# maxvonbuelow/harry

Hardware: AMD Instinct MI355X
Metric: Mtriangles/s encode+decode (higher is better)
Workload: dtype u8/u16 residual bytes, u32 range-coder registers (compat profile: u64)

## Files before the change

### harry_amd/csrc/device/chunked.cpp

```cpp
#include <chrono>
#include <condition_variable>
#include <cstdio>
#include <cstdlib>
#include <cstring>
#include <deque>
#include <memory>
#include <mutex>
#include <thread>

#include "codec_math.hpp"
#include "context.hpp"
#include "kernels.hpp"

namespace hry {

using namespace dev;
static const char kMarkPrefix[] = "[hry enc]";

static constexpr int kDefaultChunk = 8192;
static constexpr uint32_t kMaxChunk = 1u << 20;


static uint32_t stream_words(uint32_t n, uint32_t t0)
{
// ... 526 lines not shown
	shard_arrays_ready();
	const bool piped = pipe && pipe->began;
	if (pipe) { pipe->finish(); w.progress = nullptr; }
	if (piped) HRY_MARK(t_all, "  pipeline drained");
	ChunkedDirectory dir;
	std::vector<uint8_t> restart_sec;
	auto select_restarts = [&] {
		std::vector<RestartCounters> scounters;
		dir.restarts = select_restart_points(w.marks, w.named, dir.counters, &w.snapshots, &scounters);
		if (!w.snapshots.empty()) write_snapshot_section(w.snapshot_faces, w.snapshots, scounters, dir.snapshot_section);
		write_restart_section(dir, restart_sec);
	};
	const bool dir_beside = w.marks.size() >= 4096 && host_threads() > 1;
	SideThreads dir_helper;
	if (dir_beside) dir_helper.spawn(select_restarts);

	const uint32_t vc = (uint32_t)w.order_v.size(), fc = (uint32_t)w.order_f.size();
	if (piped && (vc != pipe->vc || fc != pipe->fc)) throw Error(HRY_E_INTERNAL, "encode pipeline: sizes changed under the walk");
	if (chunk_syms <= 0) {
		uint64_t total = (uint64_t)w.n_conn + (uint64_t)vc * ldv.nplanes + (uint64_t)fc * ldf.nplanes;
		if (m.general) for (const AttrList &L : m.lists) total += (uint64_t)L.count * L.coded_bytes();
		while (CH < (1u << 15) && total / CH > 8192) CH <<= 1;
	}

	auto t_h2d = Clock::now();
	size_t op_plane_n[8];
	for (int k = 0; k < 8; ++k) op_plane_n[k] = w.n_op_class[k];
	size_t ngrp = 0, conn_plane_bytes = 0, nopb = w.op_sc.size();
	for (int g = 0; g < G_COUNT; ++g) { ngrp += w.grp_val[g].size(); conn_plane_bytes += w.grp_val[g].size() * kGroupBytes[g]; }
	cx.d_order_v.ensure(std::max<size_t>((size_t)vc * 4, 16));
	cx.d_order_f.ensure(std::max<size_t>((size_t)fc * 4, 16));
	cx.d_rank.ensure(std::max<size_t>((size_t)dev_nv * 4, 16));
	cx.d_grp_val.ensure(std::max<size_t>(ngrp * 4, 16));
	cx.d_connplanes.ensure(std::max<size_t>(conn_plane_bytes + 2 * nopb + 64, 16));
	cx.d_vplanes.ensure(std::max<size_t>((size_t)vc * ldv.nplanes, 16));
	cx.d_fplanes.ensure(std::max<size_t>((size_t)fc * ldf.nplanes, 16));
	const bool nt_piped = piped && pipe->nt != nullptr;
	if (vc && !piped) HIP_OK(hipMemcpyAsync(cx.d_order_v.p, w.order_v.data(), (size_t)vc * 4, hipMemcpyHostToDevice, cx.stream));
	if (fc && (ldf.nplanes || m.general) && !piped) HIP_OK(hipMemcpyAsync(cx.d_order_f.p, w.order_f.data(), (size_t)fc * 4, hipMemcpyHostToDevice, cx.stream));
	if (!piped) upload_repaired_twins(cx, in_place ? *in_place->whole : m, w, in_place != nullptr);
	if (in_place) cx.inplace_twin_patches.insert(cx.inplace_twin_patches.end(), w.twin_patches.begin(), w.twin_patches.end());
	size_t goff[G_COUNT + 1] = { 0 };
	for (int g = 0; g < G_COUNT; ++g) {
		size_t n = w.grp_val[g].size();
		goff[g + 1] = goff[g] + n;
		if (n && !(g == G_NUMTRI && nt_piped)) HIP_OK(hipMemcpyAsync(cx.d_grp_val.as<uint32_t>() + goff[g], w.grp_val[g].data(), n * 4, hipMemcpyHostToDevice, cx.stream));
	}
	uint8_t *d_opplanes = cx.d_connplanes.as<uint8_t>() + conn_plane_bytes;
	uint8_t *d_opraw = d_opplanes + nopb;
	if (nopb) HIP_OK(hipMemcpyAsync(d_opraw, w.op_sc.data(), nopb, hipMemcpyHostToDevice, cx.stream));

	const std::vector<GenPlane> layout = container_planes(m);
	std::vector<PlaneRef> planes;
	auto add_plane = [&](const uint8_t *at, uint32_t n) { planes.push_back(PlaneRef{ at, n, layout.at(planes.size()).init }); };
	{
		size_t poff = 0;
		for (int g = 0; g < G_COUNT; ++g) {
			uint32_t n = (uint32_t)w.grp_val[g].size();
			const uint8_t *at = g == G_NUMTRI && nt_piped ? cx.d_nt_planes.as<uint8_t>() : cx.d_connplanes.as<uint8_t>() + poff;
			for (int b = 0; b < kGroupBytes[g]; ++b) add_plane(at + (size_t)b * n, n);
			poff += (size_t)n * kGroupBytes[g];
		}
		size_t o = 0;
		for (int k = 0; k < kOpClasses; ++k) { add_plane(d_opplanes + o, (uint32_t)op_plane_n[k]); o += op_plane_n[k]; }
		for (int p = 0; p < ldv.nplanes; ++p) add_plane(cx.d_vplanes.as<uint8_t>() + (size_t)p * vc, vc);
		for (int p = 0; p < ldf.nplanes; ++p) add_plane(cx.d_fplanes.as<uint8_t>() + (size_t)p * fc, fc);
	}
	if (m.general) general_planes_encode(cx, m, w, planes);
	if (planes.size() != layout.size()) throw Error(HRY_E_INTERNAL, "chunked encode: the planes do not match the container's layout");
	std::vector<uint32_t> kind_tabs;
	build_init_tables(m, kind_tabs);
	const uint32_t CHC = std::min(CH, std::max(CH / 8, 512u));
	dir.CH = CH; dir.CHC = CHC;
	const uint32_t npl = (uint32_t)planes.size();
	std::vector<HistSlice> slices;
	for (uint32_t pi = 0; pi < npl; ++pi)
		for (uint32_t f = 0; f < planes[pi].n; f += 16384) slices.push_back(HistSlice{ planes[pi].dptr + f, std::min(16384u, planes[pi].n - f), pi });
	cx.d_small.ensure(std::max<size_t>(slices.size() * sizeof(HistSlice) + (size_t)npl * 1024 + 64, 64));
	uint32_t *d_hist = cx.d_small.as<uint32_t>();
	HistSlice *d_slices = (HistSlice*)(cx.d_small.as<uint8_t>() + (size_t)npl * 1024);
	if (!slices.empty()) HIP_OK(hipMemcpyAsync(d_slices, slices.data(), slices.size() * sizeof(HistSlice), hipMemcpyHostToDevice, cx.stream));
	HIP_OK(hipMemsetAsync(d_hist, 0, (size_t)npl * 1024, cx.stream));
	HIP_OK(hipStreamSynchronize(cx.stream));
	cx.timing.h2d_ms = ms_since(t_h2d);
	HRY_MARK(t_all, "walk's outputs on the device");

	ConnView cv = cx.conn_view();
	HIP_OK(hipEventRecord(cx.ev[1], cx.stream));
	if (!m.general && !piped) {
		HIP_OK(hipMemsetAsync(cx.d_rank.p, 0xff, (size_t)dev_nv * 4, cx.stream));
		launch_rank(cx.stream, cx.d_order_v.as<uint32_t>(), vc, cv.org, cx.d_rank.as<uint32_t>());
		launch_predict_vtx(cx.stream, cv, cx.d_order_v.as<uint32_t>(), vc, cx.d_rank.as<uint32_t>(), cx.d_rec[1].as<uint8_t>(), ldv, cx.d_vplanes.as<uint8_t>());
		launch_face_planes(cx.stream, cv, cx.d_order_f.as<uint32_t>(), fc, cx.d_rec[0].as<uint8_t>(), ldf, cx.d_fplanes.as<uint8_t>());
	}
	split_conn_groups(cx, w, !nt_piped);
	{
		uint32_t base[8], o = 0;
		for (int k = 0; k < 8; ++k) { base[k] = o; o += (uint32_t)op_plane_n[k]; }
		cx.d_op.ensure(((nopb + kSplitUnit - 1) / kSplitUnit + 1) * 8 * 4 + 64);
		launch_split_classes(cx.stream, d_opraw, (uint32_t)nopb, base, cx.d_op.as<uint32_t>(), d_opplanes);
	}
	launch_plane_hist(cx.stream, d_slices, (uint32_t)slices.size(), d_hist);
	HIP_OK(hipEventRecord(cx.ev[2], cx.stream));
	std::vector<uint32_t> hist((size_t)npl * 256);
	if (npl) HIP_OK(hipMemcpyAsync(hist.data(), d_hist, hist.size() * 4, hipMemcpyDeviceToHost, cx.stream));
	HIP_OK(hipStreamSynchronize(cx.stream));
	HRY_MARK(t_all, "planes and their histograms");

	dir.tables.assign((size_t)npl * 256, 0);
	dir.has_prior.assign(npl, 0);
	dir.nsym.resize(npl);
	std::vector<uint32_t> totals(npl, 0);
	for (uint32_t pi = 0; pi < npl; ++pi) {
		uint32_t *tab = dir.tables.data() + (size_t)pi * 256;
		const bool use = plane_prior_from_hist(hist.data() + (size_t)pi * 256, planes[pi].n, tab);
		if (!use) memcpy(tab, kind_tabs.data() + (size_t)planes[pi].init * 256, 1024);
		for (int i = 0; i < 256; ++i) totals[pi] += tab[i];
		dir.has_prior[pi] = use ? 1 : 0;
		dir.nsym[pi] = planes[pi].n;
	}
	std::vector<StreamJob> jobs;
	uint64_t words = 0;
	uint64_t nsym_total = 0;
	uint32_t max_t0 = 256;
	for (uint32_t pi = 0; pi < npl; ++pi) {
		const PlaneRef &pl = planes[pi];
		nsym_total += pl.n;
		max_t0 = std::max(max_t0, totals[pi]);
		for_plane_streams(pi, pl.n, CH, CHC, [&](uint64_t f, uint32_t n) {
			if (words >= (1ull << 32) - (1u << 24)) throw Error(HRY_E_UNSUPPORTED, "chunked stream accumulator exceeds 2^32 words");
			jobs.push_back(StreamJob{ pl.dptr + f, n, pi, totals[pi], (uint32_t)words });
			words += stream_words(n, totals[pi]);
		});
	}
	const uint32_t ns = (uint32_t)jobs.size();
	const uint32_t nw = (uint32_t)words + 2;
	HRY_MARK(t_all, "  priors and stream jobs (host)");
	cx.d_init.ensure(std::max<size_t>(dir.tables.size() * 4, 16));
	if (!dir.tables.empty()) HIP_OK(hipMemcpyAsync(cx.d_init.p, dir.tables.data(), dir.tables.size() * 4, hipMemcpyHostToDevice, cx.stream));
	cx.d_cjobs.ensure(std::max<size_t>((size_t)ns * sizeof(StreamJob), 16));
	if (ns) HIP_OK(hipMemcpyAsync(cx.d_cjobs.p, jobs.data(), (size_t)ns * sizeof(StreamJob), hipMemcpyHostToDevice, cx.stream));
	cx.ensure_magic(max_t0 + CH + 16);
	cx.d_acc.ensure((size_t)nw * 8);
	cx.d_summary.ensure(((size_t)nw / 1024 + 8) * 4);
	cx.d_bytes.ensure((size_t)nw * 4);
	cx.d_csizes.ensure(std::max<size_t>((size_t)ns * 8, 16));
	cx.d_coffs.ensure(((size_t)ns + 1) * 8);
	HIP_OK(hipMemsetAsync(cx.d_acc.p, 0, (size_t)nw * 8, cx.stream));
	uint32_t *d_bits = cx.d_csizes.as<uint32_t>(), *d_nbytes = d_bits + ns;
	bool split_kernels;
	{
		uint32_t longest = 0;
		for (uint32_t i = 0; i < ns; ++i) longest = std::max(longest, jobs[i].n);
		const double one = std::max(longest * 0.09e-3, (double)nsym_total * 0.04e-6), two = longest * 0.207e-3 + (double)nsym_total * 0.0057e-6;
		const uint64_t min_streams = env_uint("HRY_ENCODE_SPLIT_MIN_STREAMS", ~0ull);
		split_kernels = min_streams != ~0ull ? min_streams != 0 && ns >= min_streams : ns >= 64 && two < 0.9 * one;
	}
	for (uint32_t i = 0; i < ns && split_kernels; ++i) split_kernels = (uint64_t)jobs[i].t0 + jobs[i].n <= 65535u;
	std::vector<uint64_t> tab;
	if (split_kernels) {
		tab.resize((size_t)ns + ((size_t)ns + 1) / 2);
		uint32_t *order = (uint32_t*)(tab.data() + ns);
		uint64_t off = 0;
		for (uint32_t i = 0; i < ns; ++i) { tab[i] = off; off += jobs[i].n; order[i] = i; }
		std::stable_sort(order, order + ns, [&](uint32_t a, uint32_t b) { return jobs[a].n > jobs[b].n; });
		cx.d_rec_sym.ensure(std::max<size_t>((size_t)off * 8, 16));
		cx.d_split.ensure(tab.size() * 8);
		HIP_OK(hipMemcpyAsync(cx.d_split.p, tab.data(), tab.size() * 8, hipMemcpyHostToDevice, cx.stream));
		HIP_OK(hipEventRecord(cx.ev[3], cx.stream));
		launch_chunk_encode_split(cx.stream, cx.d_cjobs.as<StreamJob>(), ns, cx.d_init.as<uint32_t>(), cx.d_magic.as<MagicEnt>(), cx.d_acc.as<uint64_t>(), d_bits,
		                          cx.d_split.as<uint64_t>(), cx.d_rec_sym.p, (const uint32_t*)(cx.d_split.as<uint64_t>() + ns));
		HIP_OK(hipEventRecord(cx.ev[4], cx.stream));
	} else {
	HIP_OK(hipEventRecord(cx.ev[3], cx.stream));
	launch_chunk_encode(cx.stream, cx.d_cjobs.as<StreamJob>(), ns, cx.d_init.as<uint32_t>(), cx.d_magic.as<MagicEnt>(), cx.d_acc.as<uint64_t>(), d_bits);
	HIP_OK(hipEventRecord(cx.ev[4], cx.stream));
	}
	launch_carry(cx.stream, cx.d_acc.as<uint64_t>(), nw, cx.d_v.as<uint64_t>(), cx.d_summary.as<uint32_t>(), cx.d_bytes.as<uint8_t>(), cx.d_cjobs.as<StreamJob>(), d_bits, ns);
	launch_stream_pack(cx.stream, cx.d_cjobs.as<StreamJob>(), ns, d_bits, nullptr, d_nbytes, cx.d_coffs.as<uint64_t>(), nullptr, false);
	cx.h_small.ensure(64);
	volatile uint64_t *total_bytes_p = cx.h_small.as<uint64_t>();
	*total_bytes_p = 0;
	HIP_OK(hipMemcpyAsync((void*)total_bytes_p, cx.d_coffs.as<uint64_t>() + ns, 8, hipMemcpyDeviceToHost, cx.stream));
	HRY_MARK(t_all, "  stream kernels launched");
	if (dir_beside) dir_helper.rethrow(); else select_restarts();
	HRY_MARK(t_all, "  restart points selected");
	HIP_OK(hipStreamSynchronize(cx.stream));
	const uint64_t total_bytes = *total_bytes_p;
	HRY_MARK(t_all, "streams coded");
	cx.d_cout.ensure(std::max<size_t>(total_bytes, 16));
	launch_stream_pack(cx.stream, cx.d_cjobs.as<StreamJob>(), ns, d_bits, cx.d_bytes.as<uint8_t>(), d_nbytes, cx.d_coffs.as<uint64_t>(), cx.d_cout.as<uint8_t>(), true);
	HIP_OK(hipEventRecord(cx.ev[5], cx.stream));

	write_container(cx, dir, restart_sec, ns, d_nbytes, total_bytes, out);
	HRY_MARK(t_all, "container on the host");
	if (sharded) { const uint64_t seg_len = out.size() - seg_begin; memcpy(out.data() + seg_len_at, &seg_len, 8); }
	if (cx.want_order) {
		if (sharded || in_place) throw Error(HRY_E_UNSUPPORTED, "HRY_FLAG_ORDER on a shard");
		order_build(cx, m, w, !piped ? cx.d_order_v.as<uint32_t>() : nullptr, !piped && (ldf.nplanes || m.general) ? cx.d_order_f.as<uint32_t>() : nullptr);
	}

	if (cx.keep_stages) {
		cx.stage_put_host("order_v", w.order_v.data(), (size_t)vc * 4);
		cx.stage_put_host("order_f", w.order_f.data(), (size_t)fc * 4);
		cx.stage_put("vplanes", cx.d_vplanes.p, (size_t)vc * ldv.nplanes);
		cx.stage_put("fplanes", cx.d_fplanes.p, (size_t)fc * ldf.nplanes);
		cx.stage_put("d_twin", cx.d_twin.p, (size_t)(in_place ? in_place->whole->ne() : m.ne()) * 4);
		uint64_t top = 0;
		for (uint32_t i = 0; i < ns; ++i) top = std::max(top, (uint64_t)jobs[i].t0 + jobs[i].n);
		const uint32_t plan[3] = { ns, split_kernels ? 1u : 0u, (uint32_t)top };
		cx.stage_put_host("enc_plan", plan, sizeof plan);
	}
	cx.timing.k_predict_ms = cx.elapsed(1, 2);
	cx.timing.k_entropy_ms = cx.elapsed(3, 4);
	cx.timing.device_ms = cx.elapsed(1, 5);
	cx.timing.n_symbols = nsym_total;
	cx.timing.payload_bytes = total_bytes;
	cx.timing.total_ms = ms_since(t_all);
}

Mesh *decode_chunked(Context &cx, const uint8_t *p, size_t n, size_t hdr, std::unique_ptr<Mesh> m);
Mesh *decode_compat(Context &cx, const uint8_t *p, size_t n, size_t hdr, std::unique_ptr<Mesh> m);

Mesh *decode_any(Context &cx, const uint8_t *p, size_t n, int shard_index, int shard_count, bool allow_partial)
{
	HIP_OK(hipSetDevice(cx.device));
	std::unique_ptr<Mesh> m(new Mesh());
	int minor = 0;
	const bool sharded = n >= 6 && p[4] == 0 && p[5] == 3;
	size_t hdr = read_hry_header(p, n, *m, minor, !sharded);
	if (minor == 3) { Context *one = &cx; return decode_sharded(&one, 1, p, n, hdr, std::move(m), shard_index, shard_count, allow_partial || shard_count > 1, nullptr); }
	if (shard_count > 1) throw Error(HRY_E_ARG, "only a sharded container (.hry v0.3) decodes segment by segment");
	if (minor == 2) return decode_chunked(cx, p, n, hdr, std::move(m));
	if (m->general) return decode_general(cx, p, n, hdr, std::move(m));
	return decode_compat(cx, p, n, hdr, std::move(m));
}

}
```

### harry_amd/csrc/device/chunked.hip

```cpp
#include <hip/hip_runtime.h>

#include <mutex>
#include <stdexcept>
#include <type_traits>

#include "codec_math.hpp"
#include "dev_types.hpp"
#include "kernels.hpp"
#include "wave.hpp"

namespace hry {
namespace dev {

constexpr int kWin = 72;

__global__ __launch_bounds__(64) void k_chunk_encode(const StreamJob *jobs, const uint32_t *inits, const MagicEnt *magic,
                                                     unsigned long long *acc, uint32_t *stream_bits)
{
	const StreamJob jb = jobs[blockIdx.x];
	const int lane = threadIdx.x;
	__shared__ uint32_t cnt[257], cum[257], bh[256];
	__shared__ unsigned long long win[kWin];
	{
		const uint32_t *st = inits + (size_t)jb.init * 256 + 4 * lane;
		uint32_t a = st[0], b = st[1], c = st[2], d = st[3], tot;
		uint32_t ex = wave_excl_scan(a + b + c + d, tot);
		cnt[4 * lane] = a; cnt[4 * lane + 1] = b; cnt[4 * lane + 2] = c; cnt[4 * lane + 3] = d;
		cum[4 * lane] = ex; cum[4 * lane + 1] = ex + a; cum[4 * lane + 2] = ex + a + b; cum[4 * lane + 3] = ex + a + b + c;
		if (lane == 0) { cnt[256] = 0; cum[256] = 0; }
	}
	__syncthreads();
	uint32_t R = 1u << 31;
	uint32_t S = 0;
	const uint64_t earlier = lane == 0 ? 0ull : (~0ull >> (64 - lane));
	for (uint32_t base = 0; base < jb.n; base += 64) {
		const uint32_t j = base + lane;
		const bool valid = j < jb.n;
		const uint32_t nb = min(64u, jb.n - base);
		const uint32_t s = valid ? jb.sym[j] : 0x100u;
		uint64_t eq = ~0ull, lt = 0;
#pragma unroll
		for (int b = 8; b >= 0; --b) {
			const bool mine = (s >> b) & 1u;
			const uint64_t m = __ballot(mine);
			lt |= mine ? (eq & ~m) : 0ull;
			eq &= mine ? m : ~m;
		}
		const uint32_t l = cum[s] + (uint32_t)__popcll(lt & earlier), c = cnt[s] + (uint32_t)__popcll(eq & earlier);
		const uint32_t t = jb.t0 + j;
		const bool sub = l + c == t;
		MagicEnt me = valid ? magic[t] : MagicEnt{ 0, 0, 0 };
		const uint32_t mx = valid ? (sub ? l : c) : 0u;
		const uint32_t mm = ((me.shift >> kMagicSh32Shift) & 31u) | (sub || !valid ? 0x80u : 0u);
		uint32_t my_r = 0, my_s = 0;
		const uint32_t s_first = S;
		auto step = [&](uint32_t i) {
			const uint32_t M = (uint32_t)__builtin_amdgcn_readlane((int)me.m32, (int)i);
			const uint32_t x = (uint32_t)__builtin_amdgcn_readlane((int)mx, (int)i);
			const uint32_t meta = (uint32_t)__builtin_amdgcn_readlane((int)mm, (int)i);
			const uint32_t r = __umulhi(R, M) >> (meta & 31u);
			const uint32_t prod = r * x;
			const uint32_t Rn = (meta & 0x80u) ? R - prod : prod;
			const uint32_t y = Rn - 1u;
			const uint32_t sh = y ? (uint32_t)__builtin_clz(y) - 1u : 31u;
			my_r = lane == (int)i ? r : my_r;
			my_s = lane == (int)i ? S : my_s;
			R = Rn << sh;
			S += sh;
		};
		uint32_t i = 0;
		for (; i + 4 <= nb; i += 4) { step(i); step(i + 1); step(i + 2); step(i + 3); }
		for (; i < nb; ++i) step(i);
		const uint32_t w0 = s_first >> 5, span = ((S + 63) >> 5) - w0 + 1;
		const uint32_t a = (valid && l) ? my_r * l : 0u;
		const uint32_t w = my_s >> 5, shb = my_s & 31;
		const uint32_t hi = a >> shb, lo = shb ? a << (32 - shb) : 0u;
		unsigned long long *dst = acc + jb.word_base;
		for (uint32_t k = lane; k < span; k += 64) win[k] = 0;
		bh[4 * lane] = 0; bh[4 * lane + 1] = 0; bh[4 * lane + 2] = 0; bh[4 * lane + 3] = 0;
		__syncthreads();
		if (hi) atomicAdd(&win[w - w0], (unsigned long long)hi);
		if (lo) atomicAdd(&win[w - w0 + 1], (unsigned long long)lo);
		if (valid) atomicAdd(&bh[s], 1u);
		__syncthreads();
		for (uint32_t k = lane; k < span; k += 64) {
			unsigned long long v = win[k];
			if (v) atomicAdd(&dst[w0 + k], v);
		}
		uint32_t a0 = bh[4 * lane], a1 = bh[4 * lane + 1], a2 = bh[4 * lane + 2], a3 = bh[4 * lane + 3], tot;
		uint32_t ex = wave_excl_scan(a0 + a1 + a2 + a3, tot);
		cnt[4 * lane] += a0; cnt[4 * lane + 1] += a1; cnt[4 * lane + 2] += a2; cnt[4 * lane + 3] += a3;
		cum[4 * lane] += ex; cum[4 * lane + 1] += ex + a0; cum[4 * lane + 2] += ex + a0 + a1; cum[4 * lane + 3] += ex + a0 + a1 + a2;
		__syncthreads();
	}
	if (lane == 0) stream_bits[blockIdx.x] = S + 32;
}

__global__ __launch_bounds__(64) void k_chunk_model(const StreamJob *jobs, const uint32_t *inits, const MagicEnt *magic, const unsigned long long *rec_off, uint2 *rec)
{
	const StreamJob jb = jobs[blockIdx.x];
	const int lane = threadIdx.x;
	__shared__ uint32_t cnt[257], cum[257], bh[256];
	{
		const uint32_t *st = inits + (size_t)jb.init * 256 + 4 * lane;
		uint32_t a = st[0], b = st[1], c = st[2], d = st[3], tot;
		uint32_t ex = wave_excl_scan(a + b + c + d, tot);
		cnt[4 * lane] = a; cnt[4 * lane + 1] = b; cnt[4 * lane + 2] = c; cnt[4 * lane + 3] = d;
		cum[4 * lane] = ex; cum[4 * lane + 1] = ex + a; cum[4 * lane + 2] = ex + a + b; cum[4 * lane + 3] = ex + a + b + c;
		if (lane == 0) { cnt[256] = 0; cum[256] = 0; }
	}
	__syncthreads();
	uint2 *out = rec + rec_off[blockIdx.x];
	const uint64_t earlier = lane == 0 ? 0ull : (~0ull >> (64 - lane));
	for (uint32_t base = 0; base < jb.n; base += 64) {
		const uint32_t j = base + lane;
		const bool valid = j < jb.n;
		const uint32_t s = valid ? jb.sym[j] : 0x100u;
		uint64_t eq = ~0ull, lt = 0;
#pragma unroll
		for (int b = 8; b >= 0; --b) {
			const bool mine = (s >> b) & 1u;
			const uint64_t m = __ballot(mine);
			lt |= mine ? (eq & ~m) : 0ull;
			eq &= mine ? m : ~m;
		}
		const uint32_t l = cum[s] + (uint32_t)__popcll(lt & earlier), c = cnt[s] + (uint32_t)__popcll(eq & earlier);
		if (valid) {
			const MagicEnt me = magic[jb.t0 + j];
			const uint32_t msh = (me.shift >> kMagicSh32Shift) & 31u;
			const uint32_t q = me.m32 == 0x80000000u ? me.m32 >> msh : (me.m32 - 1u) >> msh;
			out[j] = make_uint2(l | (c << 16), q);
		}
		bh[4 * lane] = 0; bh[4 * lane + 1] = 0; bh[4 * lane + 2] = 0; bh[4 * lane + 3] = 0;
		__syncthreads();
		if (valid) atomicAdd(&bh[s], 1u);
		__syncthreads();
		uint32_t a0 = bh[4 * lane], a1 = bh[4 * lane + 1], a2 = bh[4 * lane + 2], a3 = bh[4 * lane + 3], tot;
		uint32_t ex = wave_excl_scan(a0 + a1 + a2 + a3, tot);
		cnt[4 * lane] += a0; cnt[4 * lane + 1] += a1; cnt[4 * lane + 2] += a2; cnt[4 * lane + 3] += a3;
		cum[4 * lane] += ex; cum[4 * lane + 1] += ex + a0; cum[4 * lane + 2] += ex + a0 + a1; cum[4 * lane + 3] += ex + a0 + a1 + a2;
		__syncthreads();
	}
}

__global__ __launch_bounds__(64) void k_chunk_ranges(const StreamJob *jobs, uint32_t njobs, const uint32_t *order, const unsigned long long *rec_off,
                                                     const uint2 *rec, unsigned long long *acc, uint32_t *stream_bits)
{
	__shared__ uint32_t tile_lc[64 * 65], tile_q[64 * 65];
	const uint32_t lane = threadIdx.x;
	const uint32_t slot = blockIdx.x * 64 + lane;
	const bool have = slot < njobs;
	const uint32_t job = have ? order[slot] : 0u;
	StreamJob jb{ nullptr, 0, 0, 256, 0 };
	if (have) jb = jobs[job];
	const uint32_t n = have ? jb.n : 0u;
	const uint2 *in = rec + (have ? rec_off[job] : 0ull);
	unsigned long long *dst = acc + jb.word_base;
	const uint32_t nmax = (uint32_t)__builtin_amdgcn_readfirstlane((int)wave_max(n));
	const uint32_t in_lo = (uint32_t)(uintptr_t)in, in_hi = (uint32_t)((uintptr_t)in >> 32);
	uint2 nxt[64];
	auto fetch = [&](uint32_t step0) {
#pragma unroll
		for (int s = 0; s < 64; ++s) {
			const uint32_t ns = (uint32_t)__builtin_amdgcn_readlane((int)n, s);
			const uint2 *ps = (const uint2*)(((uintptr_t)(uint32_t)__builtin_amdgcn_readlane((int)in_hi, s) << 32) | (uint32_t)__builtin_amdgcn_readlane((int)in_lo, s));
			const uint32_t j = step0 + lane;
			nxt[s] = j < ns ? ps[j] : make_uint2(0u, 0u);
		}
	};
	auto stash = [&]() {
#pragma unroll
		for (int s = 0; s < 64; ++s) { tile_lc[s * 65 + lane] = nxt[s].x; tile_q[s * 65 + lane] = nxt[s].y; }
	};
	uint32_t R = 1u << 31, S = 0, t = jb.t0;
	uint32_t cur_w = 0;
	unsigned long long a0 = 0, a1 = 0;
	fetch(0);
	stash();
	for (uint32_t step0 = 0; step0 < nmax; step0 += 64) {
		const bool more = step0 + 64 < nmax;
		if (more) fetch(step0 + 64);
		const uint32_t *row_lc = tile_lc + lane * 65, *row_q = tile_q + lane * 65;
		const uint32_t left = nmax - step0 < 64u ? nmax - step0 : 64u;
		for (uint32_t k = 0; k < left; ++k) {
			const uint32_t lc = row_lc[k], q = row_q[k];
			const bool live = step0 + k < n;
			const uint32_t l = lc & 0xffffu, c = lc >> 16;
			uint32_t r = __umulhi(R, q);
			r += R - r * t >= t ? 1u : 0u;
			uint32_t rl, rc;
			asm("v_mul_lo_u32 %0, %1, %2" : "=v"(rl) : "v"(r), "v"(l));
			asm("v_mul_lo_u32 %0, %1, %2" : "=v"(rc) : "v"(r), "v"(c));
			const uint32_t Rn = l + c == t ? R - rl : rc;
			const uint32_t w = S >> 5;
			const unsigned long long two = ((unsigned long long)(live ? rl : 0u) << 32) >> (S & 31u);
			if (w != cur_w) { dst[cur_w] = a0; a0 = a1; a1 = 0; cur_w = w; }
			a0 += two >> 32;
			a1 += two & 0xffffffffull;
			const uint32_t y = Rn - 1u;
			const uint32_t sh = y ? (uint32_t)__builtin_clz(y) - 1u : 31u;
			R = live ? Rn << sh : R;
			S += live ? sh : 0u;
			t += live ? 1u : 0u;
		}
		if (more) stash();
	}
	if (have) {
		dst[cur_w] = a0;
		dst[cur_w + 1u] = a1;
		stream_bits[job] = S + 32u;
	}
}

__global__ __launch_bounds__(1024) void k_stream_offsets(const uint32_t *stream_bits, uint32_t n, uint32_t *nbytes, unsigned long long *offsets)
{
	__shared__ unsigned long long s_wave[17];
	unsigned long long carry = 0;
	for (uint32_t base = 0; base < n; base += 1024) {
		const uint32_t i = base + threadIdx.x;
		const uint32_t nb = i < n ? (stream_bits[i] + 7) >> 3 : 0;
		unsigned long long total;
		const unsigned long long ex = block_excl_scan<unsigned long long>(nb, s_wave, total);
		if (i < n) { nbytes[i] = nb; offsets[i] = carry + ex; }
		carry += total;
		__syncthreads();
	}
	if (threadIdx.x == 0) offsets[n] = carry;
}

__global__ __launch_bounds__(256) void k_pack_streams(const StreamJob *jobs, const uint8_t *bytes, const uint32_t *nbytes, const unsigned long long *offsets, uint8_t *out)
{
	const StreamJob jb = jobs[blockIdx.x];
	const uint8_t *src = bytes + (size_t)jb.word_base * 4;
	uint8_t *dst = out + offsets[blockIdx.x];
	for (uint32_t i = threadIdx.x; i < nbytes[blockIdx.x]; i += 256) dst[i] = src[i];
}

__global__ __launch_bounds__(256) void k_scatter_u8(const uint8_t *src, const uint32_t *dst_index, uint32_t n, uint8_t *dst)
{
	uint32_t i = blockIdx.x * blockDim.x + threadIdx.x;
	if (i < n) dst[dst_index[i]] = src[i];
}

__global__ __launch_bounds__(64) void k_chunk_decode(const StreamJob *jobs, const uint32_t *inits, const MagicEnt *magic,
                                                     const uint8_t *payload, const unsigned long long *offsets, const uint32_t *nbytes, uint8_t *sym_out_base)
{
	const StreamJob jb = jobs[blockIdx.x];
	const int lane = threadIdx.x;
// ... 108 lines not shown
	typedef __attribute__((address_space(1))) uint8_t gbyte;
	gbyte *out = (gbyte*)const_cast<uint8_t*>(jb.sym);
	const uint32_t nmax = (uint32_t)__builtin_amdgcn_readfirstlane((int)wave_max(jb.n));
	MagicEnt me = magic[t];
	uint32_t o0 = 0, o1 = 0, o2 = 0, o3 = 0;
	for (uint32_t i = 0; i < nmax; ++i) {
		if ((i & 15u) == 0u && i) {
			if (i < jb.n) {
				typedef uint32_t u32x4 __attribute__((ext_vector_type(4)));
				typedef __attribute__((address_space(1))) u32x4 __attribute__((aligned(1))) gvec;
				*(gvec*)(out + i - 16) = u32x4{ o0, o1, o2, o3 };
			}
		}
		if (i >= jb.n) continue;
		const uint32_t r = __umulhi(R, me.m32) >> ((me.shift >> kMagicSh32Shift) & 31u);
		me = magic[t + 1u];
		uint32_t q = (uint32_t)((float)D * __builtin_amdgcn_rcpf((float)r));
		int32_t rem = (int32_t)(D - __umul24(q, r));
		if (rem < 0) { --q; rem += (int32_t)r; }
		if (rem < 0) { --q; rem += (int32_t)r; }
		if (rem >= (int32_t)r) { ++q; rem -= (int32_t)r; }
		if (rem >= (int32_t)r) { ++q; rem -= (int32_t)r; }
		const uint32_t target = min(t - 1u, q);
		uint32_t b = 0, lo = 0;
#pragma unroll
		for (int k = 0; k < 16; ++k) {
			const bool le = C[k] <= target;
			b += le ? 1u : 0u;
			lo = le ? C[k] : lo;
		}
		const CT *cb = cnt + (size_t)(b * 16u) * 64 + lane;
		uint32_t sin = 0, run = lo, hi = 0xffffffffu;
#pragma unroll
		for (int k = 0; k < 16; ++k) {
			run += (uint32_t)cb[k * 64];
			const bool le = run <= target;
			sin += le ? 1u : 0u;
			lo = le ? run : lo;
			hi = min(hi, le ? 0xffffffffu : run);
		}
		const uint32_t s = b * 16u + sin;
		const uint32_t cs = hi - lo;
		const uint32_t rl = __umul24(r, lo);
		const uint32_t Rn = hi < t ? __umul24(r, cs) : R - rl;
		const uint32_t y = Rn - 1u;
		const uint32_t sh = y ? (uint32_t)__builtin_clz(y) - 1u : 31u;
		R = Rn << sh;
		if (avail < 32u) { buf |= (uint64_t)ahead << (32u - avail); avail += 32u; ahead = word_at(p); p += 4u; }
		const uint32_t bits = (uint32_t)((buf >> 1) >> (63u - sh));
		buf <<= sh; avail -= sh;
		D = ((D - rl) << sh) | bits;
		cnt[s * 64 + lane] = (CT)(cs + 1u);
#pragma unroll
		for (int k = 0; k < 16; ++k) C[k] += (uint32_t)k >= b ? 1u : 0u;
		++t;
		o0 = __builtin_amdgcn_alignbyte(o1, o0, 1); o1 = __builtin_amdgcn_alignbyte(o2, o1, 1); o2 = __builtin_amdgcn_alignbyte(o3, o2, 1);
		o3 = (o3 >> 8) | (s << 24);
		if (i + 1u == jb.n) {
			const uint32_t m = jb.n & 15u ? jb.n & 15u : 16u;
			auto shift = [&] { o0 = __builtin_amdgcn_alignbyte(o1, o0, 1); o1 = __builtin_amdgcn_alignbyte(o2, o1, 1); o2 = __builtin_amdgcn_alignbyte(o3, o2, 1); o3 >>= 8; };
			for (uint32_t k = m; k < 16u; ++k) shift();
			for (uint32_t k = 0; k < m; ++k) { out[jb.n - m + k] = (uint8_t)o0; shift(); }
		}
	}
}

__global__ __launch_bounds__(256) void k_scatter_u32(const uint32_t *pairs, uint32_t n, uint32_t *dst)
{
	uint32_t i = blockIdx.x * blockDim.x + threadIdx.x;
	if (i < n) dst[pairs[2 * i]] = pairs[2 * i + 1];
}

__global__ __launch_bounds__(256) void k_plane_hist(const HistSlice *slices, uint32_t *hist)
{
	const HistSlice sl = slices[blockIdx.x];
	__shared__ uint32_t bins[256];
	bins[threadIdx.x] = 0;
	__syncthreads();
	for (uint32_t i = threadIdx.x; i < sl.n; i += 256) atomicAdd(&bins[sl.sym[i]], 1u);
	__syncthreads();
	if (bins[threadIdx.x]) atomicAdd(&hist[(size_t)sl.plane * 256 + threadIdx.x], bins[threadIdx.x]);
}

__global__ __launch_bounds__(64) void k_split_count(const uint8_t *ops, uint32_t n, uint32_t *cnt)
{
	const uint32_t u = blockIdx.x, lane = threadIdx.x;
	uint32_t c[8] = { 0, 0, 0, 0, 0, 0, 0, 0 };
	for (uint32_t i = u * kSplitUnit + lane; i < min(n, (u + 1) * kSplitUnit); i += 64) {
		const uint32_t k = ops[i] >> 3;
#pragma unroll
		for (int j = 0; j < 8; ++j) c[j] += k == (uint32_t)j;
	}
#pragma unroll
	for (int j = 0; j < 8; ++j) {
		const uint32_t v = wave_sum(c[j]);
		if (lane == 0) cnt[u * 8 + j] = v;
	}
}
__global__ __launch_bounds__(64) void k_split_scan(uint32_t *cnt, uint32_t nunits, SplitBase base)
{
	const uint32_t j = blockIdx.x, lane = threadIdx.x;
	uint32_t run = base.b[j];
	for (uint32_t u0 = 0; u0 < nunits; u0 += 64) {
		const uint32_t u = u0 + lane;
		const uint32_t c = u < nunits ? cnt[u * 8 + j] : 0u;
		uint32_t tot;
		const uint32_t ex = wave_excl_scan(c, tot);
		if (u < nunits) cnt[u * 8 + j] = run + ex;
		run += tot;
	}
}
__global__ __launch_bounds__(64) void k_split_place(const uint8_t *ops, uint32_t n, const uint32_t *cnt, uint8_t *planes)
{
	const uint32_t u = blockIdx.x, lane = threadIdx.x;
	uint32_t at[8];
#pragma unroll
	for (int j = 0; j < 8; ++j) at[j] = cnt[u * 8 + j];
	const uint32_t end = min(n, (u + 1) * kSplitUnit);
	for (uint32_t i0 = u * kSplitUnit; i0 < end; i0 += 64) {
		const uint32_t i = i0 + lane;
		const bool live = i < end;
		const uint32_t b = live ? ops[i] : 0xffu, k = b >> 3;
		uint32_t dst = 0;
#pragma unroll
		for (int j = 0; j < 8; ++j) {
			const uint64_t mk = __ballot(live && k == (uint32_t)j);
			if (live && k == (uint32_t)j) dst = at[j] + (uint32_t)__popcll(mk & ((1ull << lane) - 1ull));
			at[j] += (uint32_t)__popcll(mk);
		}
		if (live) planes[dst] = (uint8_t)(b & 7u);
	}
}
void launch_split_classes(hipStream_t st, const uint8_t *ops, uint32_t n, const uint32_t base[8], uint32_t *scratch, uint8_t *planes)
{
	if (!n) return;
	const uint32_t nunits = (n + kSplitUnit - 1) / kSplitUnit;
	SplitBase sb;
	for (int j = 0; j < 8; ++j) sb.b[j] = base[j];
	hipLaunchKernelGGL(k_split_count, dim3(nunits), dim3(64), 0, st, ops, n, scratch);
	hipLaunchKernelGGL(k_split_scan, dim3(8), dim3(64), 0, st, scratch, nunits, sb);
	hipLaunchKernelGGL(k_split_place, dim3(nunits), dim3(64), 0, st, ops, n, scratch, planes);
}

void launch_plane_hist(hipStream_t st, const HistSlice *slices, uint32_t nslices, uint32_t *hist)
{
	if (nslices) hipLaunchKernelGGL(k_plane_hist, dim3(nslices), dim3(256), 0, st, slices, hist);
}
void launch_scatter_u32(hipStream_t st, const uint32_t *pairs, uint32_t n, uint32_t *dst)
{
	if (n) hipLaunchKernelGGL(k_scatter_u32, dim3((n + 255) / 256), dim3(256), 0, st, pairs, n, dst);
}
void launch_chunk_encode(hipStream_t st, const StreamJob *jobs, uint32_t nstreams, const uint32_t *inits, const MagicEnt *magic, uint64_t *acc, uint32_t *stream_bits)
{
	if (nstreams) hipLaunchKernelGGL(k_chunk_encode, dim3(nstreams), dim3(64), 0, st, jobs, inits, magic, (unsigned long long*)acc, stream_bits);
}
void launch_chunk_encode_split(hipStream_t st, const StreamJob *jobs, uint32_t nstreams, const uint32_t *inits, const MagicEnt *magic, uint64_t *acc, uint32_t *stream_bits,
                               const uint64_t *rec_off, void *rec, const uint32_t *order)
{
	if (!nstreams) return;
	hipLaunchKernelGGL(k_chunk_model, dim3(nstreams), dim3(64), 0, st, jobs, inits, magic, (const unsigned long long*)rec_off, (uint2*)rec);
	hipLaunchKernelGGL(k_chunk_ranges, dim3((nstreams + 63) / 64), dim3(64), 0, st, jobs, nstreams, order, (const unsigned long long*)rec_off, (const uint2*)rec,
	                   (unsigned long long*)acc, stream_bits);
}
void launch_stream_pack(hipStream_t st, const StreamJob *jobs, uint32_t nstreams, const uint32_t *stream_bits, const uint8_t *bytes,
                        uint32_t *nbytes, uint64_t *offsets, uint8_t *out, bool pack)
{
	if (!pack) hipLaunchKernelGGL(k_stream_offsets, dim3(1), dim3(1024), 0, st, stream_bits, nstreams, nbytes, (unsigned long long*)offsets);
	else if (nstreams) hipLaunchKernelGGL(k_pack_streams, dim3(nstreams), dim3(256), 0, st, jobs, bytes, nbytes, (const unsigned long long*)offsets, out);
}
void launch_scatter_u8(hipStream_t st, const uint8_t *src, const uint32_t *dst_index, uint32_t n, uint8_t *dst)
{
	if (n) hipLaunchKernelGGL(k_scatter_u8, dim3((n + 255) / 256), dim3(256), 0, st, src, dst_index, n, dst);
}
void launch_chunk_decode(hipStream_t st, const StreamJob *jobs, uint32_t nstreams, const uint32_t *inits, const MagicEnt *magic,
                         const uint8_t *payload, const uint64_t *offsets, const uint32_t *nbytes)
{
	if (nstreams) hipLaunchKernelGGL(k_chunk_decode, dim3(nstreams), dim3(64), 0, st, jobs, inits, magic, payload, (const unsigned long long*)offsets, nbytes, (uint8_t*)nullptr);
}
template <typename CT>
static void launch_chunk_decode_lanes_as(hipStream_t st, const StreamJob *jobs, uint32_t nstreams, const uint32_t *inits, const MagicEnt *magic,
                                         const uint8_t *payload, const uint64_t *offsets, const uint32_t *nbytes)
{
	constexpr uint32_t kLds = 256 * 64 * sizeof(CT);
	static std::mutex mu;
	static bool raised[64] = {};
	int dev = 0;
	if (hipGetDevice(&dev) != hipSuccess || dev < 0 || dev >= 64) dev = 0;
	{
		std::lock_guard<std::mutex> g(mu);
		if (!raised[dev]) {
			if (hipFuncSetAttribute((const void*)k_chunk_decode_lanes<CT>, hipFuncAttributeMaxDynamicSharedMemorySize, (int)kLds) != hipSuccess) {
				(void)hipGetLastError();
				throw std::runtime_error("k_chunk_decode_lanes: the device refuses its dynamic LDS");
			}
			raised[dev] = true;
		}
	}
	hipLaunchKernelGGL(k_chunk_decode_lanes<CT>, dim3((nstreams + 63) / 64), dim3(64), kLds, st, jobs, nstreams, inits, magic, payload, (const unsigned long long*)offsets, nbytes);
	if (hipGetLastError() != hipSuccess) throw std::runtime_error("k_chunk_decode_lanes: launch failed");
}
void launch_chunk_decode_lanes(hipStream_t st, const StreamJob *jobs, uint32_t nstreams, const uint32_t *inits, const MagicEnt *magic,
                               const uint8_t *payload, const uint64_t *offsets, const uint32_t *nbytes, bool counts16)
{
	if (!nstreams) return;
	if (counts16) launch_chunk_decode_lanes_as<uint16_t>(st, jobs, nstreams, inits, magic, payload, offsets, nbytes);
	else launch_chunk_decode_lanes_as<uint32_t>(st, jobs, nstreams, inits, magic, payload, offsets, nbytes);
}

}
}
```

Measured before the change: 64.44.

## Split fused chunk encoder into modeling and range-coding waves with software pipeline

The fused chunk encoder now runs two waves per block. One wave does symbol modeling (rank, cumulative counts, histogram update) and scatters the output bits. The other wave runs the serial range-coder recurrence, handing data through double-buffered LDS with a three-stage software pipeline. The inner range step is fully unrolled with constant-lane writelane, uses a packed op word and a branchless clz, and prefetches the next batch's symbols and reciprocals. The host split heuristic is retuned to favour the fused kernel more often, because its per-symbol cost is assumed lower. The trade-offs are more LDS, block-wide barriers per batch, and a heuristic that may now pick the fused path in cases where the split path was better.

```diff
diff --git a/harry_amd/csrc/device/chunked.cpp b/harry_amd/csrc/device/chunked.cpp
--- a/harry_amd/csrc/device/chunked.cpp
+++ b/harry_amd/csrc/device/chunked.cpp
@@ -702,7 +702,7 @@
 	{
 		uint32_t longest = 0;
 		for (uint32_t i = 0; i < ns; ++i) longest = std::max(longest, jobs[i].n);
-		const double one = std::max(longest * 0.09e-3, (double)nsym_total * 0.04e-6), two = longest * 0.207e-3 + (double)nsym_total * 0.0057e-6;
+		const double one = std::max(longest * 0.043e-3, (double)nsym_total * 0.04e-6), two = longest * 0.207e-3 + (double)nsym_total * 0.0057e-6;
 		const uint64_t min_streams = env_uint("HRY_ENCODE_SPLIT_MIN_STREAMS", ~0ull);
 		split_kernels = min_streams != ~0ull ? min_streams != 0 && ns >= min_streams : ns >= 64 && two < 0.9 * one;
 	}
diff --git a/harry_amd/csrc/device/chunked.hip b/harry_amd/csrc/device/chunked.hip
--- a/harry_amd/csrc/device/chunked.hip
+++ b/harry_amd/csrc/device/chunked.hip
@@ -14,14 +14,30 @@
 
 constexpr int kWin = 72;
 
-__global__ __launch_bounds__(64) void k_chunk_encode(const StreamJob *jobs, const uint32_t *inits, const MagicEnt *magic,
-                                                     unsigned long long *acc, uint32_t *stream_bits)
+__device__ __forceinline__ void wave_lds_order()
+{
+	__builtin_amdgcn_fence(__ATOMIC_RELEASE, "wavefront");
+	__builtin_amdgcn_wave_barrier();
+	__builtin_amdgcn_fence(__ATOMIC_ACQUIRE, "wavefront");
+}
+template <uint32_t B, uint32_t N, typename F>
+__device__ __forceinline__ void static_for(F &f)
+{
+	if constexpr (B < N) { f(std::integral_constant<uint32_t, B>()); static_for<B + 1, N>(f); }
+}
+constexpr uint32_t kOpSub = 1u << 31, kOpShift = 21, kOpX = (1u << kOpShift) - 1u;
+
+__global__ __launch_bounds__(128) void k_chunk_encode(const StreamJob *jobs, const uint32_t *inits, const MagicEnt *magic,
+                                                      unsigned long long *acc, uint32_t *stream_bits)
 {
 	const StreamJob jb = jobs[blockIdx.x];
-	const int lane = threadIdx.x;
+	const int lane = threadIdx.x & 63;
+	const bool ranger = __builtin_amdgcn_readfirstlane((int)(threadIdx.x >> 6)) != 0;
 	__shared__ uint32_t cnt[257], cum[257], bh[256];
 	__shared__ unsigned long long win[kWin];
-	{
+	__shared__ uint32_t op_m[2][64], op_x[2][64];
+	__shared__ uint32_t rs_r[2][64], rs_s[2][64], rs_end[2];
+	if (!ranger) {
 		const uint32_t *st = inits + (size_t)jb.init * 256 + 4 * lane;
 		uint32_t a = st[0], b = st[1], c = st[2], d = st[3], tot;
 		uint32_t ex = wave_excl_scan(a + b + c + d, tot);
@@ -29,71 +45,110 @@
 		cum[4 * lane] = ex; cum[4 * lane + 1] = ex + a; cum[4 * lane + 2] = ex + a + b; cum[4 * lane + 3] = ex + a + b + c;
 		if (lane == 0) { cnt[256] = 0; cum[256] = 0; }
 	}
-	__syncthreads();
+	const uint32_t nbatch = (jb.n + 63u) >> 6;
 	uint32_t R = 1u << 31;
 	uint32_t S = 0;
 	const uint64_t earlier = lane == 0 ? 0ull : (~0ull >> (64 - lane));
-	for (uint32_t base = 0; base < jb.n; base += 64) {
-		const uint32_t j = base + lane;
-		const bool valid = j < jb.n;
-		const uint32_t nb = min(64u, jb.n - base);
-		const uint32_t s = valid ? jb.sym[j] : 0x100u;
-		uint64_t eq = ~0ull, lt = 0;
-#pragma unroll
-		for (int b = 8; b >= 0; --b) {
-			const bool mine = (s >> b) & 1u;
-			const uint64_t m = __ballot(mine);
-			lt |= mine ? (eq & ~m) : 0ull;
-			eq &= mine ? m : ~m;
-		}
-		const uint32_t l = cum[s] + (uint32_t)__popcll(lt & earlier), c = cnt[s] + (uint32_t)__popcll(eq & earlier);
-		const uint32_t t = jb.t0 + j;
-		const bool sub = l + c == t;
-		MagicEnt me = valid ? magic[t] : MagicEnt{ 0, 0, 0 };
-		const uint32_t mx = valid ? (sub ? l : c) : 0u;
-		const uint32_t mm = ((me.shift >> kMagicSh32Shift) & 31u) | (sub || !valid ? 0x80u : 0u);
-		uint32_t my_r = 0, my_s = 0;
-		const uint32_t s_first = S;
-		auto step = [&](uint32_t i) {
-			const uint32_t M = (uint32_t)__builtin_amdgcn_readlane((int)me.m32, (int)i);
-			const uint32_t x = (uint32_t)__builtin_amdgcn_readlane((int)mx, (int)i);
-			const uint32_t meta = (uint32_t)__builtin_amdgcn_readlane((int)mm, (int)i);
-			const uint32_t r = __umulhi(R, M) >> (meta & 31u);
-			const uint32_t prod = r * x;
-			const uint32_t Rn = (meta & 0x80u) ? R - prod : prod;
-			const uint32_t y = Rn - 1u;
-			const uint32_t sh = y ? (uint32_t)__builtin_clz(y) - 1u : 31u;
-			my_r = lane == (int)i ? r : my_r;
-			my_s = lane == (int)i ? S : my_s;
-			R = Rn << sh;
-			S += sh;
-		};
-		uint32_t i = 0;
-		for (; i + 4 <= nb; i += 4) { step(i); step(i + 1); step(i + 2); step(i + 3); }
-		for (; i < nb; ++i) step(i);
-		const uint32_t w0 = s_first >> 5, span = ((S + 63) >> 5) - w0 + 1;
-		const uint32_t a = (valid && l) ? my_r * l : 0u;
-		const uint32_t w = my_s >> 5, shb = my_s & 31;
-		const uint32_t hi = a >> shb, lo = shb ? a << (32 - shb) : 0u;
-		unsigned long long *dst = acc + jb.word_base;
-		for (uint32_t k = lane; k < span; k += 64) win[k] = 0;
-		bh[4 * lane] = 0; bh[4 * lane + 1] = 0; bh[4 * lane + 2] = 0; bh[4 * lane + 3] = 0;
+	const uint2 *recip = (const uint2*)magic + 1;
+	auto fetch = [&](uint32_t b, uint32_t &s, uint2 &me) {
+		const uint32_t j = b * 64u + lane;
+		const bool valid = !ranger && j < jb.n;
+		s = valid ? jb.sym[j] : 0x100u;
+		me = valid ? recip[2 * (size_t)(jb.t0 + j)] : make_uint2(0u, 0u);
+	};
+	uint32_t s_nx, l1 = 0, l2 = 0;
+	uint2 me_nx;
+	fetch(0, s_nx, me_nx);
+	unsigned long long *dst = acc + jb.word_base;
+	__syncthreads();
+	for (uint32_t p = 0; p < nbatch + 2; ++p) {
+		if (!ranger) {
+			const uint32_t s = s_nx;
+			const uint2 me = me_nx;
+			if (p + 1 < nbatch) fetch(p + 1, s_nx, me_nx);
+			if (p >= 2) {
+				const uint32_t q = p & 1u;
+				const uint32_t my_r = rs_r[q][lane], my_s = rs_s[q][lane];
+				const uint32_t s_first = (uint32_t)__builtin_amdgcn_readfirstlane((int)my_s), s_end = rs_end[q];
+				const uint32_t w0 = s_first >> 5, span = ((s_end + 63) >> 5) - w0 + 1;
+				const uint32_t a = l2 ? my_r * l2 : 0u;
+				const uint32_t w = my_s >> 5, shb = my_s & 31;
+				const uint32_t hi = a >> shb, lo = shb ? a << (32 - shb) : 0u;
+				for (uint32_t k = lane; k < span; k += 64) win[k] = 0;
+				wave_lds_order();
+				if (hi) atomicAdd(&win[w - w0], (unsigned long long)hi);
+				if (lo) atomicAdd(&win[w - w0 + 1], (unsigned long long)lo);
+				wave_lds_order();
+				for (uint32_t k = lane; k < span; k += 64) {
+					unsigned long long v = win[k];
+					if (v) atomicAdd(&dst[w0 + k], v);
+				}
+				wave_lds_order();
+			}
+			l2 = l1;
+			l1 = 0;
+			if (p < nbatch) {
+				const uint32_t j = p * 64u + lane;
+				const bool valid = j < jb.n;
+				uint64_t eq = ~0ull, lt = 0;
+#pragma unroll
+				for (int b = 8; b >= 0; --b) {
+					const bool mine = (s >> b) & 1u;
+					const uint64_t m = __ballot(mine);
+					lt |= mine ? (eq & ~m) : 0ull;
+					eq &= mine ? m : ~m;
+				}
+				const uint32_t l = cum[s] + (uint32_t)__popcll(lt & earlier), c = cnt[s] + (uint32_t)__popcll(eq & earlier);
+				const uint32_t t = jb.t0 + j;
+				const bool sub = l + c == t;
+				const uint32_t x = valid ? (sub ? l : c) : 0u;
+				op_m[p & 1u][lane] = me.y;
+				op_x[p & 1u][lane] = x | (sub ? kOpSub : 0u) | (((me.x >> kMagicSh32Shift) & 31u) << kOpShift);
+				l1 = valid ? l : 0u;
+				bh[4 * lane] = 0; bh[4 * lane + 1] = 0; bh[4 * lane + 2] = 0; bh[4 * lane + 3] = 0;
+				wave_lds_order();
+				if (valid) atomicAdd(&bh[s], 1u);
+				wave_lds_order();
+				uint32_t a0 = bh[4 * lane], a1 = bh[4 * lane + 1], a2 = bh[4 * lane + 2], a3 = bh[4 * lane + 3], tot;
+				uint32_t ex = wave_excl_scan(a0 + a1 + a2 + a3, tot);
+				cnt[4 * lane] += a0; cnt[4 * lane + 1] += a1; cnt[4 * lane + 2] += a2; cnt[4 * lane + 3] += a3;
+				cum[4 * lane] += ex; cum[4 * lane + 1] += ex + a0; cum[4 * lane + 2] += ex + a0 + a1; cum[4 * lane + 3] += ex + a0 + a1 + a2;
+				wave_lds_order();
+			}
+		} else if (p >= 1 && p <= nbatch) {
+			const uint32_t q = (p - 1u) & 1u;
+			const uint32_t nb = min(64u, jb.n - (p - 1u) * 64u);
+			const uint32_t vm = op_m[q][lane], vx = op_x[q][lane];
+			uint32_t my_r = 0, my_s = 0;
+			auto step = [&](auto i) {
+				const uint32_t M = (uint32_t)__builtin_amdgcn_readlane((int)vm, (int)i);
+				const uint32_t ox = (uint32_t)__builtin_amdgcn_readlane((int)vx, (int)i);
+				const uint32_t r = __umulhi(R, M) >> ((ox >> kOpShift) & 31u);
+				const uint32_t prod = r * (ox & kOpX);
+				const uint32_t Rn = (int32_t)ox < 0 ? R - prod : prod;
+				const uint32_t sh = (uint32_t)__builtin_clz((Rn << 1) - 1u);
+				if constexpr (std::is_integral<decltype(i)>::value) {
+					my_r = lane == (int)i ? r : my_r;
+					my_s = lane == (int)i ? S : my_s;
+				} else {
+					asm("v_writelane_b32 %0, %1, %2" : "+v"(my_r) : "s"(r), "n"(decltype(i)::value));
+					asm("v_writelane_b32 %0, %1, %2" : "+v"(my_s) : "s"(S), "n"(decltype(i)::value));
+				}
+				R = Rn << sh;
+				S += sh;
+			};
+			if (nb == 64u) {
+				static_for<0, 64>(step);
+			} else {
+				for (uint32_t i = 0; i < nb; ++i) step(i);
+			}
+			rs_r[q][lane] = my_r;
+			rs_s[q][lane] = my_s;
+			if (lane == 0) rs_end[q] = S;
+		}
 		__syncthreads();
-		if (hi) atomicAdd(&win[w - w0], (unsigned long long)hi);
-		if (lo) atomicAdd(&win[w - w0 + 1], (unsigned long long)lo);
-		if (valid) atomicAdd(&bh[s], 1u);
-		__syncthreads();
-		for (uint32_t k = lane; k < span; k += 64) {
-			unsigned long long v = win[k];
-			if (v) atomicAdd(&dst[w0 + k], v);
-		}
-		uint32_t a0 = bh[4 * lane], a1 = bh[4 * lane + 1], a2 = bh[4 * lane + 2], a3 = bh[4 * lane + 3], tot;
-		uint32_t ex = wave_excl_scan(a0 + a1 + a2 + a3, tot);
-		cnt[4 * lane] += a0; cnt[4 * lane + 1] += a1; cnt[4 * lane + 2] += a2; cnt[4 * lane + 3] += a3;
-		cum[4 * lane] += ex; cum[4 * lane + 1] += ex + a0; cum[4 * lane + 2] += ex + a0 + a1; cum[4 * lane + 3] += ex + a0 + a1 + a2;
-		__syncthreads();
-	}
-	if (lane == 0) stream_bits[blockIdx.x] = S + 32;
+	}
+	if (threadIdx.x == 64) stream_bits[blockIdx.x] = S + 32;
 }
 
 __global__ __launch_bounds__(64) void k_chunk_model(const StreamJob *jobs, const uint32_t *inits, const MagicEnt *magic, const unsigned long long *rec_off, uint2 *rec)
@@ -508,7 +563,7 @@
 }
 void launch_chunk_encode(hipStream_t st, const StreamJob *jobs, uint32_t nstreams, const uint32_t *inits, const MagicEnt *magic, uint64_t *acc, uint32_t *stream_bits)
 {
-	if (nstreams) hipLaunchKernelGGL(k_chunk_encode, dim3(nstreams), dim3(64), 0, st, jobs, inits, magic, (unsigned long long*)acc, stream_bits);
+	if (nstreams) hipLaunchKernelGGL(k_chunk_encode, dim3(nstreams), dim3(128), 0, st, jobs, inits, magic, (unsigned long long*)acc, stream_bits);
 }
 void launch_chunk_encode_split(hipStream_t st, const StreamJob *jobs, uint32_t nstreams, const uint32_t *inits, const MagicEnt *magic, uint64_t *acc, uint32_t *stream_bits,
                                const uint64_t *rec_off, void *rec, const uint32_t *order)
```

New measurement: 62.56. 2.9% lower.
